# JGCRI/xanthos

Measured on AMD Instinct MI355X. Metric: cell-months/sec (pm_abcd_mrtm, 67,420 cells), higher is better.
Workload: dtype f64

## Files before the change

xanthos_amd/csrc/xh_mrtm_rsum.hip:

```cpp
#include <algorithm>
#include "xh_mrtm_wave_unit.h"

namespace {

__global__ void __launch_bounds__(LANES) __attribute__((amdgpu_waves_per_eu(2, 2))) k_mrtm_rsum(const WaveArgs *ap_) {
    WaveArgsK *ap = (WaveArgsK *)ap_;
    __shared__ __attribute__((aligned(16))) v2d lds[RING * NSLOT];
    __shared__ uint2 xtab[LANES];
    __shared__ unsigned qstage_sh[4 * LANES];
    __shared__ double fend_sh[2 * LANES];
    __shared__ int unit_sh, prio_sh;
    const int unit = wave_claim(ap, &unit_sh, &prio_sh);
    const int prio = prio_sh;
    if (unit < 0) return;
    if (A(months_ready)) {
        if (prio == 3) __builtin_amdgcn_s_setprio(3);
        else if (prio == 1) __builtin_amdgcn_s_setprio(1);
        else __builtin_amdgcn_s_setprio(2);
    } else if (prio == 3) {
        __builtin_amdgcn_s_setprio(3);
    }
    const int p = A(unit_p)[unit];
    const bool has_ghost = A(ghost_edge)[(int64_t)unit * LANES + threadIdx.x] >= 0;
    const bool g = __any(has_ghost), g2 = __any(has_ghost && threadIdx.x >= 8);
    const int nxo = __popcll(__ballot(A(export_edge)[(int64_t)unit * LANES + threadIdx.x] >= 0));
    const bool x = nxo > 0;
    char *l = reinterpret_cast<char *>(lds);
    __attribute__((address_space(3))) unsigned *qst = (__attribute__((address_space(3))) unsigned *)qstage_sh;
    __attribute__((address_space(3))) double *fnd = (__attribute__((address_space(3))) double *)fend_sh;
    fend_sh[threadIdx.x] = 0.0;
    fend_sh[LANES + threadIdx.x] = 0.0;
    if ((p & ~31) != 0x400) {
        if (threadIdx.x == 0) __hip_atomic_store(A(fault), FAULT_PLACE_WAIT, __ATOMIC_RELAXED, __HIP_MEMORY_SCOPE_AGENT);
        return;
    }
    bool bad = false;
#define XH_BY_OUTLETS(...)                                                                 \
    do {                                                                                   \
        if (nxo > 8) wave_unit<__VA_ARGS__, -1>(ap, l, xtab, qst, fnd, unit);              \
        else if (x) wave_unit<__VA_ARGS__, 1>(ap, l, xtab, qst, fnd, unit);                \
        else wave_unit<__VA_ARGS__, 0>(ap, l, xtab, qst, fnd, unit);                       \
    } while (0)
    if (p & 16) {
        if (!(p & 8) || (p & 4)) bad = true;
        else if (g2) XH_BY_OUTLETS(1, 0, 2, true, true, false, 2);
        else if (g) XH_BY_OUTLETS(1, 0, 1, true, true, false, 2);
        else XH_BY_OUTLETS(1, 0, 0, true, true, false, 2);
#undef XH_BY_OUTLETS
    } else if (p & 8) {
        if (p & 4) {
            if (g || !A(fold_cell)) bad = true;
            else wave_unit<1, 0, 0, true, true, true, 1>(ap, l, xtab, qst, fnd, unit);
        } else if (g2) wave_unit<1, 0, 2, true, true, false, 1>(ap, l, xtab, qst, fnd, unit);
        else if (g) wave_unit<1, 0, 1, true, true, false, 1>(ap, l, xtab, qst, fnd, unit);
        else if ((p & 2) || x) wave_unit<1, 0, 0, true, true, false, 1>(ap, l, xtab, qst, fnd, unit);
        else if (p & 1) wave_unit<1, 0, 0, false, true, false, 1>(ap, l, xtab, qst, fnd, unit);
        else wave_unit<0, 0, 0, false, true, false, 1>(ap, l, xtab, qst, fnd, unit);
    } else if (p & 4) {
        if (g || !A(fold_cell)) bad = true;
        else wave_unit<1, 0, 0, true, true, true>(ap, l, xtab, qst, fnd, unit);
    } else if (g2) wave_unit<1, 0, 2, true, true>(ap, l, xtab, qst, fnd, unit);
    else if (g) wave_unit<1, 0, 1, true, true>(ap, l, xtab, qst, fnd, unit);
    else if ((p & 2) || x) wave_unit<1, 0, 0, true, true>(ap, l, xtab, qst, fnd, unit);
    else if (p & 1) wave_unit<1, 0, 0, false, true>(ap, l, xtab, qst, fnd, unit);
    else wave_unit<0, 0, 0, false, true>(ap, l, xtab, qst, fnd, unit);
    if (bad && threadIdx.x == 0)
        __hip_atomic_store(A(fault), FAULT_PLACE_WAIT, __ATOMIC_RELAXED, __HIP_MEMORY_SCOPE_AGENT);
}
#undef A

}

const void *wave_rsum_kernel() { return reinterpret_cast<const void *>(&k_mrtm_rsum); }
```

xanthos_amd/csrc/xh_mrtm_wave.hip:

```cpp
#include <algorithm>
#include "xh_mrtm_wave_unit.h"

namespace {

__global__ void __launch_bounds__(LANES) __attribute__((amdgpu_waves_per_eu(2, 2))) k_mrtm_wave(const WaveArgs *ap_) {
    WaveArgsK *ap = (WaveArgsK *)ap_;
    __shared__ __attribute__((aligned(16))) v2d lds[RING * NSLOT];
    __shared__ uint2 xtab[LANES];
    __shared__ unsigned qstage_sh[2 * LANES];
    __shared__ double fend_sh[LANES];
    __shared__ int unit_sh, prio_sh;
    const int unit = wave_claim(ap, &unit_sh, &prio_sh);
    const int prio = prio_sh;
    if (unit < 0) return;
    if (A(months_ready)) {
        if (prio == 3) __builtin_amdgcn_s_setprio(3);
        else if (prio == 1) __builtin_amdgcn_s_setprio(1);
        else __builtin_amdgcn_s_setprio(2);
    } else if (prio == 3) {
        __builtin_amdgcn_s_setprio(3);
    }
    const int p = A(unit_p)[unit];
    const bool has_ghost = A(ghost_edge)[(int64_t)unit * LANES + threadIdx.x] >= 0;
    const bool g = __any(has_ghost), g2 = __any(has_ghost && threadIdx.x >= 8);
    char *l = reinterpret_cast<char *>(lds);
    __attribute__((address_space(3))) unsigned *qst = (__attribute__((address_space(3))) unsigned *)qstage_sh;
    __attribute__((address_space(3))) double *fnd = (__attribute__((address_space(3))) double *)fend_sh;
    fend_sh[threadIdx.x] = 0.0;
#define WAVE_FORM(PRE, POST, CHAINED, NG1)                                                        \
    case (PRE) | ((POST) << 4) | ((CHAINED) ? 0x100 : 0):                                         \
        if (g2 || (g && !(NG1))) wave_unit<PRE, POST, 2, CHAINED>(ap, l, xtab, qst, fnd, unit);        \
        else if (g) wave_unit<PRE, POST, (NG1) ? 1 : 2, CHAINED>(ap, l, xtab, qst, fnd, unit);         \
        else wave_unit<PRE, POST, 0, CHAINED>(ap, l, xtab, qst, fnd, unit);                            \
        break;
#define WAVE_PAIR(PRE, POST, CHAINED) WAVE_FORM(PRE, POST, CHAINED, false)
#define WAVE_PAIR1(PRE, POST, CHAINED) WAVE_FORM(PRE, POST, CHAINED, true)
    switch (p) {
        WAVE_PAIR1(1, 1, false) WAVE_PAIR1(1, 2, false) WAVE_PAIR1(1, 3, false) WAVE_PAIR1(1, 4, false)
        WAVE_PAIR(2, 1, false) WAVE_PAIR1(2, 2, false) WAVE_PAIR1(2, 3, false) WAVE_PAIR1(2, 4, false)
        WAVE_PAIR(3, 1, false) WAVE_PAIR1(3, 2, false) WAVE_PAIR(3, 3, false) WAVE_PAIR(3, 4, false)
        WAVE_PAIR(4, 1, false) WAVE_PAIR(4, 2, false) WAVE_PAIR(4, 3, false) WAVE_PAIR(4, 4, false)
        WAVE_PAIR(1, 1, true) WAVE_PAIR1(1, 2, true) WAVE_PAIR1(1, 3, true) WAVE_PAIR(1, 4, true)
        WAVE_PAIR(2, 1, true) WAVE_PAIR1(2, 2, true) WAVE_PAIR1(2, 3, true) WAVE_PAIR(2, 4, true)
        default:
            if (threadIdx.x == 0) __hip_atomic_store(A(fault), FAULT_PLACE_WAIT, __ATOMIC_RELAXED, __HIP_MEMORY_SCOPE_AGENT);
    }
#undef WAVE_PAIR1
#undef WAVE_PAIR
#undef WAVE_FORM
}
#undef A

}

const void *wave_exact_kernel() { return reinterpret_cast<const void *>(&k_mrtm_wave); }
```

xanthos_amd/csrc/xh_mrtm_wave_launch.hip:

```cpp
#include <algorithm>
#include "xh_mrtm_wave_unit.h"
#undef A

namespace {

__global__ void k_mrtm_wave_args(WaveArgs a, WaveArgs *dst, uint4 *cnt, unsigned cnt_vec) {
    if (threadIdx.x == 0) *dst = a;
    if (threadIdx.x == 0 && a.months_ready)
        __hip_atomic_store(const_cast<unsigned *>(a.months_ready), a.ready_at_launch, __ATOMIC_RELAXED, __HIP_MEMORY_SCOPE_AGENT);
    for (unsigned i = threadIdx.x; i < cnt_vec; i += blockDim.x) cnt[i] = make_uint4(0u, 0u, 0u, 0u);
}

}

int wave_launch(xh_ctx *ctx, FlowPlan *fp, const FlowSched &s, const FlowIO &io, hipStream_t st, unsigned **place) {
    if (!fp || fp->n_units == 0) return XH_OK;
    if (!fp->skew_ok || fp->max_imports > 8 * SK_R || fp->max_exports > 8 * SK_R || s.ntmin < fp->skew_lmax + 2 * GROUP) {
        if (xh_flow_debug())
            fprintf(stderr, "time-skewed kernel not used: skew_ok %d, imports %d, outlets %d, shortest month %d sub-steps, largest lag %d\n",
                    (int)fp->skew_ok, fp->max_imports, fp->max_exports, s.ntmin, fp->skew_lmax);
        return XH_ERR_LIMIT;
    }
    {
        uint64_t limit = (uint64_t)1 << 32;
// ... 2 lines not shown
        if ((uint64_t)(fp->max_cell + 1) * stride > limit || (io.feed && (int64_t)fp->max_cell >= io.feed->ncell)) {
            if (xh_flow_debug())
                fprintf(stderr, "round-3 time-skewed kernel not used: %d rows x %d months x 8 B exceed its 32-bit row offsets\n",
                        fp->max_cell + 1, s.nmonths);
            return XH_ERR_LIMIT;
        }
    }
    int rs = 2048;
    while (rs < 8 * CH + 4 * fp->skew_lmax || rs < 1024 + (2 * CH + 256) * fp->skew_span) rs *= 2;
    if (const char *env = getenv("XH_FLOW_RS")) {
        const int v = atoi(env);
        if (v >= 2048 && (v & (v - 1)) == 0) rs = v;
    }
    const size_t x_streams = (size_t)std::max(fp->n_edges, 1) * (size_t)rs * sizeof(v2d);
    if (x_streams + (size_t)rs * 16 > ((size_t)1 << 32)) return XH_ERR_LIMIT;
    const size_t x_cnt = ((size_t)(fp->n_edges + fp->n_units + PLACE_WORDS) * sizeof(unsigned) + 255) & ~size_t(255);
    const size_t x_rec0 = ((size_t)(s.nit + 3) * sizeof(MonthRec) + 255) & ~size_t(255);
    const size_t x_rec = x_rec0 + (((size_t)(s.nit + 2) * sizeof(FinRec) + 255) & ~size_t(255));
    if (x_streams + x_cnt + x_rec > fp->x_bytes) {
        if (fp->d_x) {
            XH_HIP(ctx, hipStreamSynchronize(st));
            XH_HIP(ctx, hipFree(fp->d_x));
            fp->d_x = nullptr;
        }
        XH_HIP(ctx, hipMalloc(&fp->d_x, x_streams + x_cnt + x_rec));
        fp->x_bytes = x_streams + x_cnt + x_rec;
        fp->rec_key = 0;
    }
    unsigned *cnt = reinterpret_cast<unsigned *>(static_cast<char *>(fp->d_x) + x_streams);
    MonthRec *d_rec = reinterpret_cast<MonthRec *>(static_cast<char *>(fp->d_x) + x_streams + x_cnt);
    FinRec *d_fin = reinterpret_cast<FinRec *>(static_cast<char *>(fp->d_x) + x_streams + x_cnt + x_rec0);
    const FlowFeed *feed = io.feed;
    auto q_off = [&](int m) -> long long {
        if (!feed) return (long long)m * 8;
        return (long long)(m >> 4) * feed->ncell * 128 + (long long)(m & 15) * 8;
    };
    uint64_t rec_key = XH_FNV_BASIS;
    {
        const long long lay[4] = {s.nit, s.total, feed ? (long long)feed->ncell : -1ll, (long long)(size_t)fp->d_x};
        rec_key = xh_fnv1a(rec_key, lay, sizeof(lay));
        rec_key = xh_fnv1a(rec_key, s.h_m, sizeof(int) * (size_t)s.nit);
        rec_key = xh_fnv1a(rec_key, s.h_nt, sizeof(int) * (size_t)s.nit);
        rec_key = xh_fnv1a(rec_key, s.h_g, sizeof(int) * (size_t)(s.nit + 1));
        rec_key = xh_fnv1a(rec_key, s.h_wr, (size_t)s.nit);
        rec_key = xh_fnv1a(rec_key, s.h_secs, sizeof(double) * (size_t)s.nit);
        if (rec_key == 0) rec_key = 1;
    }
    if (rec_key != fp->rec_key) {
        fp->rec_key = 0;
        fp->h_rec.assign((size_t)(s.nit + 3) * sizeof(MonthRec), 0);
        MonthRec *h = reinterpret_cast<MonthRec *>(fp->h_rec.data());
        for (int it = 0; it < s.nit; ++it) {
            h[it].m = s.h_m[it];
            h[it].nt = s.h_nt[it];
            h[it].g = s.h_g[it];
            h[it].write = s.h_wr[it];
            h[it].secs = s.h_secs[it];
            h[it].q_off = q_off(s.h_m[it]);
        }
        h[s.nit].g = s.total;
        fp->h_fin.assign((size_t)(s.nit + 2) * sizeof(FinRec), 0);
        FinRec *hf = reinterpret_cast<FinRec *>(fp->h_fin.data());
        for (int it = 0; it <= s.nit; ++it) {
            if (it >= 1) {
                hf[it].m_prev_w = h[it - 1].m | (h[it - 1].write ? FIN_WRITE : 0);
                hf[it].nt_prev = h[it - 1].nt;
            }
            hf[it].nt_prev = std::max(hf[it].nt_prev, 1);
            hf[it].secs_next1 = it + 1 < s.nit ? h[it + 1].secs : 1.0;
            hf[it].m_next2 = it + 2 < s.nit ? h[it + 2].m : 0;
            hf[it].q_off_next2 = q_off(hf[it].m_next2);
            hf[it].g_next1 = it + 1 <= s.nit ? h[it + 1].g : s.total;
        }
        hf[s.nit + 1].nt_prev = 1;
        hf[s.nit + 1].secs_next1 = 1.0;
        XH_HIP(ctx, hipMemcpyAsync(d_rec, h, fp->h_rec.size(), hipMemcpyHostToDevice, st));
        XH_HIP(ctx, hipMemcpyAsync(d_fin, hf, fp->h_fin.size(), hipMemcpyHostToDevice, st));
        fp->rec_key = rec_key;
    }

    const int cus = ctx->prop.multiProcessorCount > 0 ? ctx->prop.multiProcessorCount : 256;
    const void *kernel = fp->rsum ? wave_rsum_kernel() : wave_exact_kernel();
    const size_t lds_static = (size_t)RING * NSLOT * sizeof(v2d) + LANES * sizeof(uint2) + 2 * LANES * sizeof(unsigned) +
                              LANES * sizeof(double) + 64 +
                              (fp->rsum ? 2 * LANES * sizeof(unsigned) + LANES * sizeof(double) : 0);
    int n_excl = 0;
    if (fp->rsum && fp->n_special >= 0 && fp->n_pair_units > 0 && xh_env_on("XH_RSUM_EXCL", true))
        n_excl = std::min(fp->n_pair_units, 0xffff);
    int n_wg = 0, resident = 0;
    size_t lds = 0;
    {
        n_wg = fp->n_units + cus;
        if (n_wg > 8 * cus) n_wg = std::max(fp->n_units, 8 * cus);
        {
            const char *env = getenv("XH_FLOW_SPARE");
            if (env) n_wg = fp->n_units + std::max(atoi(env), 0);
        }
        const int per_cu = (n_wg + cus - 1) / cus + 3;
        const size_t share = ((size_t)(160 * 1024) / (size_t)per_cu) & ~size_t(1023);
        lds = share > lds_static + 1024 ? share - lds_static : 0;
        XH_HIP(ctx, hipFuncSetAttribute(kernel, hipFuncAttributeMaxDynamicSharedMemorySize, (int)lds));
        XH_HIP(ctx, hipOccupancyMaxActiveBlocksPerMultiprocessor(&resident, kernel, LANES, lds));
        if ((int64_t)(resident - 1) * cus < n_wg || n_wg > 8 * cus) return XH_ERR_LIMIT;
    }

    WaveArgs a;
    a.cell_of_slot = static_cast<const int *>(fp->d_cell_of_slot.p);
    a.lag = static_cast<const int *>(fp->d_lag.p);
    a.ghost_lag = static_cast<const int *>(fp->d_ghost_lag.p);
    a.export_edge = static_cast<const int *>(fp->d_export_edge.p);
    a.ghost_edge = static_cast<const int *>(fp->d_ghost_edge.p);
    a.edge_cons_unit = static_cast<const int *>(fp->d_edge_cons_unit.p);
    a.ent2 = static_cast<const unsigned *>(fp->d_ent2.p);
    a.eprev = static_cast<const unsigned *>(fp->d_eprev.p);
    a.unit_p = static_cast<const int *>(fp->d_unit_p.p);
    a.unit_order = static_cast<const int *>(fp->d_unit_order.p);
    a.n_units = fp->n_units;
    a.unit_lmax = static_cast<const int *>(fp->d_unit_lmax.p);
    a.unit_glmax = static_cast<const int *>(fp->d_unit_glmax.p);
    a.total_slots = (int64_t)fp->n_units * LANES;
    a.nmonths = s.nmonths;
    a.nit = s.nit;
    a.total = s.total;
    a.odd_ok = s.nt_even ? 0 : 1;
    a.rec = d_rec;
    a.fin = d_fin;
    a.lane_flags = static_cast<const unsigned char *>(fp->d_lane_flags.p);
    a.dt = s.dt;
    a.dtinv = 1.0 / s.dt;
    a.flow_dist = io.flow_dist;
    a.velocity = io.velocity;
    a.area = io.area;
    a.runoff = feed ? feed->q_staged : io.runoff;
    a.q_row_stride = feed ? 128u : (unsigned)s.nmonths * 8u;
    a.ready_at_launch = feed ? feed->ready_at_launch : UINT_MAX;
    a.months_ready = feed ? feed->months_ready : nullptr;
    a.place_epoch = feed ? feed->place_epoch : nullptr;
    a.epoch = feed ? feed->epoch : 0u;
    a.n_excl = n_excl;
    a.fenced = xh_env_on("XH_ROUTE_FENCED", false) ? 1 : 0;
    a.S0 = io.S0;
    a.chs = io.chs;
    a.avg = io.avg;
    a.S_end = io.S_end;
    a.F_end = io.F_end;
    a.xbuf = static_cast<char *>(fp->d_x);
    a.xbytes = (unsigned)x_streams;
    a.ring_mask_b = (unsigned)rs * 16u - 1u;
    a.rs = rs;
    a.ready = cnt;
    a.done = cnt + fp->n_edges;
    a.place = cnt + fp->n_edges + fp->n_units;
    *place = a.place;
    unsigned *fault = nullptr;
    int rc = xh_fault_word(ctx, &fault);
    if (rc) return rc;
    a.fault = fault;
    if (s.test_fault) XH_HIP(ctx, hipMemsetD32Async(reinterpret_cast<hipDeviceptr_t>(fault), (int)FAULT_TEST, 1, st));
    a.stats = nullptr;
    {
        const char *env = getenv("XH_FLOW_STATS");
        if (env && env[0] == '1') {
            if (!fp->d_stats) XH_HIP(ctx, hipMalloc(reinterpret_cast<void **>(&fp->d_stats), (size_t)fp->n_units * 48));
            a.stats = fp->d_stats;
        }
    }
    a.fold_cell = static_cast<const int *>(fp->d_fold_cell.p);
// ... 12 lines not shown
```

xanthos_amd/csrc/xh_mrtm_wave_unit.h:

```cpp
#pragma once
#include <algorithm>
#include <climits>
#include <cstdlib>
#include <type_traits>

#include "xh_mrtm_flow.h"

namespace {


constexpr int LANES = 64;
constexpr int SK_P = 4;
#ifndef XH_WAVE_MIDZONE
#define XH_WAVE_MIDZONE 1
#endif
#ifndef XH_WAVE_BMOV
#define XH_WAVE_BMOV 1
#endif
constexpr int NSLOT = 2 * LANES + 1;
constexpr int RING = 8;
constexpr int GROUP = 16;
constexpr int SK_R = 2;
#ifndef XH_WAVE_CH
#define XH_WAVE_CH 256
// ... 36 lines not shown
    int odd_ok;
    const MonthRec *rec;
    const FinRec *fin;
    double dt, dtinv;
    const double *flow_dist, *velocity, *area, *runoff, *S0;
    double *chs, *avg, *S_end, *F_end;
    unsigned q_row_stride;
    unsigned ready_at_launch;
    const unsigned *months_ready;
    unsigned *place_epoch;
    unsigned epoch;
    int n_excl;
    int fenced;
    char *xbuf;
    unsigned xbytes;
    unsigned ring_mask_b;
    int rs;
    unsigned *ready;
    unsigned *done;
    unsigned *fault;
    unsigned long long *stats;
    const int *fold_cell;
};

__device__ __forceinline__ unsigned ld_relaxed(const unsigned *p) {
    return __hip_atomic_load(p, __ATOMIC_RELAXED, __HIP_MEMORY_SCOPE_AGENT);
}

constexpr unsigned long long SPIN_LIMIT_TICKS = 500000000ull;

__device__ __forceinline__ bool wave_wait_ge(bool need, const unsigned *p, unsigned target, unsigned &seen,
                                             unsigned *fault, unsigned code) {
    bool ok = !need || seen >= target;
    if (__all(ok)) return true;
    const unsigned long long t0 = __builtin_amdgcn_s_memrealtime();
    for (;;) {
        if (!ok) {
            seen = ld_relaxed(p);
            ok = seen >= target;
        }
        if (__all(ok)) return true;
        if (ld_relaxed(fault) != 0) return false;
        if (__builtin_amdgcn_s_memrealtime() - t0 > SPIN_LIMIT_TICKS) {
            __hip_atomic_store(fault, code, __ATOMIC_RELAXED, __HIP_MEMORY_SCOPE_AGENT);
            return false;
        }
        __builtin_amdgcn_s_sleep(4);
    }
}

typedef double v2d __attribute__((ext_vector_type(2)));
typedef unsigned v4u __attribute__((ext_vector_type(4)));
constexpr int AUX_SC1 = 16;
typedef __attribute__((address_space(3))) const char lds_cchar;
typedef __attribute__((address_space(3))) char lds_char;

typedef __attribute__((address_space(4))) const WaveArgs WaveArgsK;
template <class T>
__device__ __forceinline__ T xh_ldarg(__attribute__((address_space(4))) const T *p) {
    asm volatile("" : "+s"(p));
    return *p;
}
#define A(f) xh_ldarg(&ap->f)

template <bool ONE> struct Val;
template <> struct Val<false> {
    typedef v2d T;
    typedef __attribute__((address_space(3))) const v2d lds_c;
    typedef __attribute__((address_space(3))) v2d lds_m;
    static constexpr unsigned B = 16;
    static __device__ __forceinline__ T zero() { return v2d{0.0, 0.0}; }
};
template <> struct Val<true> {
    typedef double T;
    typedef __attribute__((address_space(3))) const double lds_c;
    typedef __attribute__((address_space(3))) double lds_m;
    static constexpr unsigned B = 8;
    static __device__ __forceinline__ T zero() { return 0.0; }
};

template <int PRE, int POST, int NG, bool CHAIN, bool RSUM = false, bool FOLD = false, int SGL = 0, int NXR = -1>
__device__ __forceinline__ void wave_unit(WaveArgsK *ap, char *lds_generic, uint2 *xtab,
                                          __attribute__((address_space(3))) unsigned *qstage,
                                          __attribute__((address_space(3))) double *fend, const int unit) {
    constexpr bool HAS_G = NG > 0;
    constexpr bool V8 = SGL == 1;
    typedef Val<V8> V;
    typedef typename V::T val_t;
    typedef typename V::lds_c lds_cv;
    typedef typename V::lds_m lds_mv;
    constexpr unsigned VB = V::B;
    constexpr unsigned SLOTB = NSLOT * VB;
    lds_char *lds0 = (lds_char *)lds_generic;
    const int lane = threadIdx.x;
    const int64_t slot = (int64_t)unit * LANES + lane;

    const int gc = A(cell_of_slot)[slot];
    const bool valid = gc >= 0;
    const int gc_safe = valid ? gc : 0;
    const unsigned row_off = (unsigned)gc_safe * A(q_row_stride);
    const double tauinv = valid ? A(velocity)[gc] / A(flow_dist)[gc] : 0.0;
    const double acoef = 1.0 - tauinv * A(dt);
    const double area = valid ? A(area)[gc] : 0.0;
    const double S0v = (valid && A(S0)) ? A(S0)[gc] : 0.0;
    auto ent_off = [](unsigned o) { return V8 ? o >> 1 : o; };
    static_assert(!RSUM || (PRE <= 1 && POST == 0), "reassociated form: one inflow entry");
    static_assert(!FOLD || (RSUM && NG == 0), "folded leaves: reassociated form, units without imports");
    static_assert(SGL == 0 || RSUM, "single-sum plans: reassociated form");
    const int gcL = FOLD ? A(fold_cell)[slot] : -1;
    const bool validL = FOLD && valid && gcL >= 0;
    const unsigned row_offL = (unsigned)(validL ? gcL : 0) * A(q_row_stride);
    const double tauL = validL ? A(velocity)[gcL] / A(flow_dist)[gcL] : 0.0;
    const double acoefL = 1.0 - tauL * A(dt);
    const double areaL = validL ? A(area)[gcL] : 0.0;
    const double S0L = (validL && A(S0)) ? A(S0)[gcL] : 0.0;
    double SL = 0.0, favgL = 0.0, erlL = 0.0, erlL_n = 0.0, snapSL = 0.0, snapAL = 0.0, FL = 0.0;
    constexpr double FOLD_EPS = 1e-6;
    unsigned gfold = (validL && !(tauL * A(dt) <= 1.0 - 1.0 / 1048576.0 && tauL >= 0.0 && S0L >= 0.0)) ? 1u : 0u;
    constexpr double SGL_EPS = 1e-6;
    constexpr double SGL_XEPS = 1e-10;
    unsigned gsgl = 0;
    bool xlane = false;
    double fmin_seen = 0.0;
    if (SGL != 0) {
        const unsigned lf = A(lane_flags)[slot];
        xlane = valid && (lf & 2u) != 0;
        gsgl = (valid && (!(tauinv >= 0.0) || (!(tauinv * A(dt) <= 1.0 - 1.0 / 1048576.0) && !(lf & 1u)) || S0v < 0.0)) ? 1u : 0u;
    }
    constexpr int PRE_N = PRE > 0 ? PRE : 1, POST_N = POST > 0 ? POST : 1;
    lds_cchar *epre[PRE_N], *epost[POST_N];
#pragma unroll
    for (int w = 0; w < PRE; ++w) epre[w] = lds0 + ent_off(A(ent2)[(int64_t)w * A(total_slots) + slot]);
#pragma unroll
    for (int w = 0; w < POST; ++w) epost[w] = lds0 + ent_off(A(ent2)[(int64_t)(SK_P + w) * A(total_slots) + slot]);
    lds_cchar *eprv = lds0 + (CHAIN ? ent_off(A(eprev)[slot]) : 0u);
    lds_mv *own = (lds_mv *)lds0 + lane;
    const int xedge = A(export_edge)[slot];
    const int gedge = A(ghost_edge)[slot];
    const bool has_x = xedge >= 0, has_g = gedge >= 0;
    const unsigned long long xmask = __ballot(has_x), gmask = __ballot(has_g);
    const int nx_out = __popcll(xmask), ng = __popcll(gmask);
    static_assert(NXR >= -1 && NXR <= 1, "outlet rounds known at compile time: none or one");
    const bool any_x = NXR < 0 ? xmask != 0 : NXR > 0, any_g = HAS_G;
    const int lmax = A(unit_lmax)[unit], glmax = A(unit_glmax)[unit];
    const int lag_g = has_g ? A(ghost_lag)[slot] : 0;
    const unsigned *ready_p = A(ready) + (has_g ? gedge : 0);
    const unsigned *done_p = A(done) + (has_x ? A(edge_cons_unit)[xedge] : 0);
    const unsigned maskb = A(ring_mask_b);
    const unsigned oob = ~maskb;
    const __amdgpu_buffer_rsrc_t xr = __builtin_amdgcn_make_buffer_rsrc(A(xbuf), 0, (int)A(xbytes), 0x00020000);
    const int total = A(total), nit = A(nit);
    const bool odd_ok = A(odd_ok) != 0;

    if (has_x) xtab[__popcll(xmask & ((1ull << lane) - 1ull))] = make_uint2((unsigned)lane, (unsigned)xedge);
    const int sub = lane & 7, grp = lane >> 3;
    const bool x2 = NXR < 0 && nx_out > 8;
    unsigned gfull[SK_R], xbyte[SK_R];
    lds_mv *gdst[SK_R];
    lds_cv *xsrc[SK_R];
#pragma unroll
    for (int r = 0; r < SK_R; ++r) {
        const int k = r * 8 + grp;
        const bool gon = k < ng, xon = k < nx_out;
        const int ge = gon ? A(ghost_edge)[(int64_t)unit * LANES + k] : 0;
        const int gl = gon ? A(ghost_lag)[(int64_t)unit * LANES + k] : 0;
        gfull[r] = gon ? ((unsigned)ge * (maskb + 1u)) | (((unsigned)(sub - gl) * 16u) & maskb) : oob;
// ... 34 lines not shown
        MonthRec r;
        r.m = p_rec[i].m;
        r.nt = p_rec[i].nt;
        r.g = p_rec[i].g;
        r.write = p_rec[i].write;
        r.secs = p_rec[i].secs;
        r.q_off = p_rec[i].q_off;
        return r;
    };
    const int nmo = A(nmonths);
    const unsigned q_lds = (unsigned)(size_t)qstage;
    auto runoff_fetch = [&](long long q_off) {
        const char *src = reinterpret_cast<const char *>(p_runoff) + q_off + (size_t)row_off;
        unsigned keep;
        asm volatile("s_mov_b32 %0, m0\n\ts_mov_b32 m0, %2\n\tglobal_load_lds_dword %1, off\n\ts_add_u32 m0, m0, 252\n\t"
                     "global_load_lds_dword %1, off offset:4\n\ts_mov_b32 m0, %0"
                     : "=&s"(keep)
                     : "v"(src), "s"(q_lds)
                     : "memory");
        if (FOLD) {
            const char *srcL = reinterpret_cast<const char *>(p_runoff) + q_off + (size_t)row_offL;
            asm volatile("s_mov_b32 %0, m0\n\ts_mov_b32 m0, %2\n\tglobal_load_lds_dword %1, off\n\ts_add_u32 m0, m0, 252\n\t"
                         "global_load_lds_dword %1, off offset:4\n\ts_mov_b32 m0, %0"
                         : "=&s"(keep)
                         : "v"(srcL), "s"(q_lds + 2u * LANES * 4u)
                         : "memory");
        }
    };
    auto runoff_take = [&]() {
        if (any_x || any_g) asm volatile("s_waitcnt vmcnt(4)" ::: "memory");
        else asm volatile("s_waitcnt vmcnt(0)" ::: "memory");
        const unsigned lo = qstage[lane], hi = qstage[LANES + lane];
        return __hiloint2double((int)hi, (int)lo);
    };
    double erl_n = 0.0;
    {
        const MonthRec r0 = ld_rec(0), r1 = ld_rec(1);
        auto ld_q = [&](long long q_off) {
            return *reinterpret_cast<const double *>(reinterpret_cast<const char *>(p_runoff) + q_off + (size_t)row_off);
        };
        const double q0 = ld_q(r0.q_off);
        erl_n = ((valid ? q0 : 0.0) * area) * 1000.0 / r0.secs;
        if (RSUM) erl_n *= A(dt);
        if (SGL != 0) gsgl |= (erl_n < -SGL_EPS) ? 2u : 0u;
        if (FOLD) {
            const double q0L = *reinterpret_cast<const double *>(reinterpret_cast<const char *>(p_runoff) + r0.q_off + (size_t)row_offL);
            erlL_n = (((validL ? q0L : 0.0) * areaL) * 1000.0 / r0.secs) * A(dt);
        }
        if (nit > 1) runoff_fetch(r1.q_off);
    }
    constexpr int OB = 4;
    double ob_s[OB], ob_a[OB];
    double ob_sL[FOLD ? OB : 1], ob_aL[FOLD ? OB : 1];
#pragma unroll
    for (int j = 0; j < OB; ++j) ob_s[j] = ob_a[j] = 0.0;
#pragma unroll
    for (int j = 0; j < (FOLD ? OB : 1); ++j) ob_sL[j] = ob_aL[j] = 0.0;
    bool alive = true;
    unsigned mready = A(ready_at_launch);
    auto wait_months = [&](unsigned need) {
        const unsigned *p = A(months_ready);
        if (!p) return true;
        const unsigned long long t0 = __builtin_amdgcn_s_memrealtime();
        for (;;) {
            unsigned v = 0;
            if (lane == 0) v = __hip_atomic_fetch_add(const_cast<unsigned *>(p), 0u, __ATOMIC_RELAXED, __HIP_MEMORY_SCOPE_AGENT);
            v = (unsigned)__builtin_amdgcn_readfirstlane((int)v);
            if (v >= need) {
                mready = v;
                return true;
            }
            if (ld_relaxed(A(fault)) != 0) return false;
            if (__builtin_amdgcn_s_memrealtime() - t0 > SPIN_LIMIT_TICKS) {
                __hip_atomic_store(A(fault), FAULT_DATA_WAIT, __ATOMIC_RELAXED, __HIP_MEMORY_SCOPE_AGENT);
                return false;
            }
            __builtin_amdgcn_s_sleep(16);
        }
    };
    unsigned long long cyc_wait_data = 0, cyc_wait_ring = 0, zone_groups = 0;
    const unsigned long long cyc_begin = __builtin_amdgcn_s_memtime();
    const unsigned long long rt_begin = __builtin_amdgcn_s_memrealtime();

    unsigned seen_ready = 0, seen_done = 0, pend_ready = 0, pend_done = 0;
    auto load_async = [&](const unsigned *q) {
        unsigned v;
        asm volatile("global_load_dword %0, %1, off sc1" : "=v"(v) : "v"(q) : "memory");
        return v;
    };
    auto check = [&](int n) {
        const unsigned long long w0 = __builtin_amdgcn_s_memtime();
        asm volatile("s_waitcnt vmcnt(8)" : "+v"(pend_ready), "+v"(pend_done) : : "memory");
        asm volatile("s_waitcnt vmcnt(0)" ::: "memory");
        if (SGL == 2) gsgl |= (xlane && fmin_seen < -SGL_XEPS) ? 4u : 0u;
        if ((FOLD && __any(gfold != 0)) || (SGL != 0 && __any(gsgl != 0))) {
            __hip_atomic_store(A(fault), FAULT_GUARD, __ATOMIC_RELAXED, __HIP_MEMORY_SCOPE_AGENT);
            alive = false;
        }
        const bool fenced = A(fenced) == 1;
        if (any_x) {
            const int pub = min(max(n - RING - lmax, 0), total);
            if (fenced) __builtin_amdgcn_fence(__ATOMIC_RELEASE, "agent");
            if (has_x) __hip_atomic_store(A(ready) + xedge, (unsigned)pub, __ATOMIC_RELAXED, __HIP_MEMORY_SCOPE_AGENT);
            const int need = n + CH - lmax - A(rs);
            seen_done = max(seen_done, pend_done);
            if (need > 0 && alive)
                alive = wave_wait_ge(has_x, done_p, (unsigned)min(need, total), seen_done, A(fault), FAULT_RING_WAIT);
        }
        const unsigned long long w1 = __builtin_amdgcn_s_memtime();
        if (any_g && alive) {
            if (lane == 0)
                __hip_atomic_store(A(done) + unit, (unsigned)min(max(n - glmax, 0), total), __ATOMIC_RELAXED,
                                   __HIP_MEMORY_SCOPE_AGENT);
            const int need = min(total, n + CH + GROUP - lag_g);
            seen_ready = max(seen_ready, pend_ready);
            alive = wave_wait_ge(has_g && need > 0, ready_p, (unsigned)max(need, 0), seen_ready, A(fault), FAULT_DATA_WAIT);
            if (fenced) __builtin_amdgcn_fence(__ATOMIC_ACQUIRE, "agent");
            asm volatile("" ::: "memory");
        }
        if (any_x) pend_done = load_async(done_p);
        if (any_g) pend_ready = load_async(ready_p);
        cyc_wait_ring += w1 - w0;
        cyc_wait_data += __builtin_amdgcn_s_memtime() - w1;
    };

    auto finalize = [&](int it) {
        const FinRec f = fc;
        fc = ld_fin(it + 1 <= nit ? it + 1 : nit + 1);
        if (it + 1 < nit) {
            const double qn = runoff_take();
            erl_n = ((valid ? qn : 0.0) * area) * 1000.0 / f.secs_next1;
            if (RSUM) erl_n *= dt;
            if (SGL != 0) gsgl |= (erl_n < -SGL_EPS) ? 2u : 0u;
            if (FOLD) {
                const unsigned lo = qstage[2 * LANES + lane], hi = qstage[3 * LANES + lane];
                const double qnL = __hiloint2double((int)hi, (int)lo);
                erlL_n = (((validL ? qnL : 0.0) * areaL) * 1000.0 / f.secs_next1) * dt;
            }
        }
        if (it >= 1) {
            const int m = f.m_prev_w & (FIN_WRITE - 1);
            const bool write_prev = (f.m_prev_w & FIN_WRITE) != 0;
#pragma unroll
            for (int j = 0; j < OB - 1; ++j) {
                ob_s[j] = ob_s[j + 1];
                ob_a[j] = ob_a[j + 1];
            }
            ob_s[OB - 1] = snapS;
            ob_a[OB - 1] = snapA / (double)f.nt_prev;
            if (FOLD) {
#pragma unroll
                for (int j = 0; j < OB - 1; ++j) {
                    ob_sL[j] = ob_sL[j + 1];
                    ob_aL[j] = ob_aL[j + 1];
                }
                ob_sL[OB - 1] = snapSL;
                ob_aL[OB - 1] = snapAL / (double)f.nt_prev;
                gfold |= (snapSL < -FOLD_EPS) ? 2u : 0u;
                if (write_prev && validL) {
                    if ((m & (OB - 1)) == OB - 1) {
                        const int64_t o = (int64_t)gcL * nmo + (m - (OB - 1));
#pragma unroll
                        for (int j = 0; j < OB; j += 2) {
                            if (p_chs) *reinterpret_cast<v2d *>(p_chs + o + j) = v2d{ob_sL[j], ob_sL[j + 1]};
                            if (p_avg) *reinterpret_cast<v2d *>(p_avg + o + j) = v2d{ob_aL[j], ob_aL[j + 1]};
                        }
                    } else if (m == nmo - 1) {
                        const int r = (m & (OB - 1)) + 1;
                        const int64_t o = (int64_t)gcL * nmo + (m + 1 - r);
#pragma unroll
                        for (int j = 0; j < OB; ++j)
                            if (j >= OB - r) {
                                if (p_chs) p_chs[o + j - (OB - r)] = ob_sL[j];
                                if (p_avg) p_avg[o + j - (OB - r)] = ob_aL[j];
                            }
                    }
                }
            }
            if (write_prev && valid) {
                if ((m & (OB - 1)) == OB - 1) {
                    const int64_t o = (int64_t)gc * nmo + (m - (OB - 1));
#pragma unroll
                    for (int j = 0; j < OB; j += 2) {
                        if (p_chs) *reinterpret_cast<v2d *>(p_chs + o + j) = v2d{ob_s[j], ob_s[j + 1]};
                        if (p_avg) *reinterpret_cast<v2d *>(p_avg + o + j) = v2d{ob_a[j], ob_a[j + 1]};
                    }
                } else if (m == nmo - 1) {
                    const int r = (m & (OB - 1)) + 1;
                    const int64_t o = (int64_t)gc * nmo + (m + 1 - r);
#pragma unroll
                    for (int j = 0; j < OB; ++j)
                        if (j >= OB - r) {
                            if (p_chs) p_chs[o + j - (OB - r)] = ob_s[j];
                            if (p_avg) p_avg[o + j - (OB - r)] = ob_a[j];
                        }
                }
            }
        }
        if (it + 2 < nit) {
            if ((unsigned)f.m_next2 >= mready) alive = wait_months((unsigned)f.m_next2 + 1u);
            if (alive) runoff_fetch(f.q_off_next2);
        }
        return f.g_next1;
    };
// ... 180 lines not shown
    }
    unsigned long long prof_plain = 0;
#else
#define PROF_MARK(acc)
#endif
    auto housekeeping = [&](int n) {
        if (n > 0 && (n & (CH - 1)) == 0) check(n);
        if (alive && n == nf) {
            const int g_next = finalize(itf);
            ++itf;
            nf = itf <= nit ? ((g_next + lmax + 1 + GROUP - 1) & ~(GROUP - 1)) : INT_MAX;
        }
        PROF_MARK(prof_fin)
    };
    int n = 0;
    while (n < N && alive) {
        if (itz <= nit && n + GROUP > gz && n <= gz + lmax) {
            const int edge = itz == 0 ? 1 : (itz == nit ? 2 : 0);
            auto zone_run = [&](auto mid_c) {
                do {
                    housekeeping(n);
                    if (!alive) break;
                    ++zone_groups;
                    const int rel = nx - n;
#pragma unroll
                    for (int j = 0; j < GROUP; ++j) substep(std::true_type(), mid_c, n, j, edge, rel);
                    n += GROUP;
                    PROF_MARK(prof_zone)
                } while (n <= gz + lmax && n < N);
            };
#if XH_WAVE_MIDZONE
            if (edge == 0 && !odd_ok) zone_run(std::true_type());
            else zone_run(std::false_type());
#else
            zone_run(std::false_type());
#endif
            if (alive) {
                nx = itz < nit ? nx + ntz : INT_MAX;
                ++itz;
                gz = p_rec[itz <= nit ? itz : nit].g;
                if (itz > nit) gz = INT_MAX;
                ntz = p_rec[itz <= nit ? itz : nit].nt;
            }
        } else {
            const int n_end = itz <= nit ? min(N, gz & ~(GROUP - 1)) : N;
            do {
                housekeeping(n);
                if (!alive) break;
#pragma unroll
                for (int j = 0; j < GROUP; ++j) substep(std::false_type(), std::false_type(), n, j, 0, 0);
                n += GROUP;
                PROF_MARK(prof_plain)
            } while (n < n_end);
        }
    }
    if (alive) {
        while (itf <= nit) finalize(itf++);
        if (SGL == 2) gsgl |= (xlane && fmin_seen < -SGL_XEPS) ? 4u : 0u;
        if ((FOLD && __any(gfold != 0)) || (SGL != 0 && __any(gsgl != 0))) {
            __hip_atomic_store(A(fault), FAULT_GUARD, __ATOMIC_RELAXED, __HIP_MEMORY_SCOPE_AGENT);
            alive = false;
        }
    }
    if (alive) {
        if (any_x) {
            const unsigned xpos = ((unsigned)(N - RING - lmax) * 16u) & maskb;
            store_pair(*xsrc[0], xbyte[0], xpos);
            if (x2) store_pair(*xsrc[1], xbyte[1], xpos);
            asm volatile("s_waitcnt vmcnt(0)" ::: "memory");
            if (A(fenced) == 1) __builtin_amdgcn_fence(__ATOMIC_RELEASE, "agent");
            if (has_x) __hip_atomic_store(A(ready) + xedge, (unsigned)total, __ATOMIC_RELAXED, __HIP_MEMORY_SCOPE_AGENT);
        }
        if (any_g && lane == 0)
            __hip_atomic_store(A(done) + unit, (unsigned)total, __ATOMIC_RELAXED, __HIP_MEMORY_SCOPE_AGENT);
        if (valid) {
            if (A(S_end)) A(S_end)[gc] = snapS;
            if (A(F_end)) A(F_end)[gc] = fend[lane];
        }
        if (validL) {
            if (A(S_end)) A(S_end)[gcL] = snapSL;
            if (A(F_end)) A(F_end)[gcL] = fend[LANES + lane];
        }
    }
    const bool guard_set = __any((gfold | gsgl) != 0);
    if (A(stats) && lane == 0) {
        unsigned long long *st = A(stats) + (int64_t)unit * 6;
        const unsigned long long cyc = __builtin_amdgcn_s_memtime() - cyc_begin;
        st[0] = cyc - cyc_wait_data - cyc_wait_ring;
        st[1] = cyc;
        st[2] = __builtin_amdgcn_s_memrealtime() - rt_begin;
        const unsigned hw = __builtin_amdgcn_s_getreg((4) | (0 << 6) | (31 << 11));
        const unsigned xcc = __builtin_amdgcn_s_getreg((20) | (0 << 6) | (3 << 11));
        st[3] = (unsigned long long)((PRE + POST + (CHAIN ? 1 : 0) + 1) & 15) | (any_g ? 16u : 0u) | (any_x ? 32u : 0u) |
                (V8 ? 64u : 0u) | (guard_set ? 128u : 0u) | ((unsigned long long)hw << 8) | ((unsigned long long)(xcc & 15u) << 40) |
                (zone_groups << 44);
        st[4] = cyc_wait_data;
        st[5] = cyc_wait_ring;
#ifdef XH_WAVE_PROFILE
        st[0] = prof_plain;
        st[4] = prof_zone;
        st[5] = prof_fin;
#endif
    }
}


__device__ __forceinline__ int wave_claim(WaveArgsK *ap, int *unit_sh_p, int *prio_sh_p) {
    int &unit_sh = *unit_sh_p, &prio_sh = *prio_sh_p;
    if (threadIdx.x == 0) {
        prio_sh = 0;
        unsigned *pl = A(place);
        const unsigned hw = __builtin_amdgcn_s_getreg((4) | (0 << 6) | (31 << 11));
        const unsigned xcc = __builtin_amdgcn_s_getreg((20) | (0 << 6) | (3 << 11)) & 15u;
        const unsigned key = ((((xcc * 8u + ((hw >> 13) & 7u)) * 2u + ((hw >> 12) & 1u)) * 16u + ((hw >> 8) & 15u)) * 4u) +
                             ((hw >> 4) & 3u);
        unsigned *pl_cu = pl + 16 + PLACE_KEYS + (key >> 2);
        const int n_units = A(n_units);
        const unsigned n_wg = gridDim.x;
        unsigned *fault = A(fault);
        auto wait_for = [&](unsigned *word, unsigned target) {
            const unsigned long long t0 = __builtin_amdgcn_s_memrealtime();
            while (__hip_atomic_load(word, __ATOMIC_ACQUIRE, __HIP_MEMORY_SCOPE_AGENT) < target) {
                if (ld_relaxed(fault) != 0 || __builtin_amdgcn_s_memrealtime() - t0 > SPIN_LIMIT_TICKS) {
                    __hip_atomic_store(fault, FAULT_PLACE_WAIT, __ATOMIC_RELAXED, __HIP_MEMORY_SCOPE_AGENT);
                    return false;
                }
                __builtin_amdgcn_s_sleep(8);
            }
            return true;
        };
        auto add = [&](int word) { return __hip_atomic_fetch_add(pl + word, 1u, __ATOMIC_RELAXED, __HIP_MEMORY_SCOPE_AGENT); };
        const unsigned rank = __hip_atomic_fetch_add(pl + 16 + key, 1u, __ATOMIC_RELAXED, __HIP_MEMORY_SCOPE_AGENT) & 0xffffu;
        bool leader = false;
        unsigned cu_rank = 0;
        if (rank == 0) {
            add(2);
            cu_rank = __hip_atomic_fetch_add(pl_cu, 1u, __ATOMIC_RELAXED, __HIP_MEMORY_SCOPE_AGENT) & 0xffffu;
            leader = cu_rank == 0u;
            if (leader) add(9);
        } else if (rank == 1) {
            add(1);
        }
        const unsigned registered = __hip_atomic_fetch_add(pl + 0, 1u, __ATOMIC_RELEASE, __HIP_MEMORY_SCOPE_AGENT);
        if (registered + 1u == n_wg && A(place_epoch))
            __hip_atomic_store(A(place_epoch), A(epoch), __ATOMIC_RELAXED, __HIP_MEMORY_SCOPE_AGENT);
        int idx = -1;
        if (wait_for(pl + 0, n_wg)) {
            const int firsts = (int)ld_relaxed(pl + 2), seconds = (int)ld_relaxed(pl + 1), leaders = (int)ld_relaxed(pl + 9);
            const int n_excl = A(n_excl);
            int ncu = min(n_excl, leaders);
            ncu = max(min(ncu, (seconds - max(n_units - firsts, 0)) / 7), 0);
            bool excl_cu = false;
            int displaced = 0, claimed = 0;
            bool ok = true;
            if (ncu > 0) {
                if (leader) {
                    if ((int)add(10) < ncu) {
                        const int cnt = (int)(ld_relaxed(pl_cu) & 0xffffu);
                        const int base = (int)add(13);
                        if (base < n_excl) {
                            __hip_atomic_fetch_or(pl_cu, 0x10000u, __ATOMIC_RELAXED, __HIP_MEMORY_SCOPE_AGENT);
                            __hip_atomic_fetch_add(pl + 11, (unsigned)(cnt - 1), __ATOMIC_RELAXED, __HIP_MEMORY_SCOPE_AGENT);
                            idx = n_units - 1 - base;
                        }
                    }
                    __hip_atomic_fetch_add(pl + 12, 1u, __ATOMIC_RELEASE, __HIP_MEMORY_SCOPE_AGENT);
                }
                ok = wait_for(pl + 12, (unsigned)leaders);
                excl_cu = (ld_relaxed(pl_cu) & 0x10000u) != 0;
                displaced = (int)ld_relaxed(pl + 11);
                claimed = min((int)ld_relaxed(pl + 13), n_excl);
            }
            const int nx = claimed;
            const int firsts_eff = firsts - displaced;
            const int need2 = max(n_units - firsts_eff, 0);
            if (idx >= 0 || !ok) {
            } else if (rank >= 2) {
                idx = -2;
// ... 31 lines not shown
```

Baseline: 3.176 billion.

## Stage async progress-counter loads through LDS and specialize single-unit rsum outlets

The asynchronous polls of the neighbour ready/done counters now use global_load_lds_dword into a new LDS staging buffer, not VGPR-returning loads, which frees registers and removes the inline-asm register ties that held them live across the wait. The check step reads the staged values back from LDS, and a final vmcnt(0) drain is added before exit. Separately, the rsum kernel now also dispatches single-group (SGL=1) units through the outlet-count specializations, which adds template instantiations and code size. The LDS staging adds M0 save/restore overhead and a small LDS footprint, and the static-LDS size accounting is updated to match.

```diff
diff --git a/xanthos_amd/csrc/xh_mrtm_rsum.hip b/xanthos_amd/csrc/xh_mrtm_rsum.hip
--- a/xanthos_amd/csrc/xh_mrtm_rsum.hip
+++ b/xanthos_amd/csrc/xh_mrtm_rsum.hip
@@ -1,5 +1,13 @@
 #include <algorithm>
 #include "xh_mrtm_wave_unit.h"
+
+#define XH_SGL_FOLD 1
+#define XH_SGL_NG0 2
+#define XH_SGL_NG1 4
+#define XH_SGL_NG2 8
+#ifndef XH_RSUM_SGL_NXR
+#define XH_RSUM_SGL_NXR (XH_SGL_FOLD | XH_SGL_NG0 | XH_SGL_NG1 | XH_SGL_NG2)
+#endif
 
 namespace {
 
@@ -8,6 +16,7 @@
     __shared__ __attribute__((aligned(16))) v2d lds[RING * NSLOT];
     __shared__ uint2 xtab[LANES];
     __shared__ unsigned qstage_sh[4 * LANES];
+    __shared__ unsigned cstage_sh[2 * LANES];
     __shared__ double fend_sh[2 * LANES];
     __shared__ int unit_sh, prio_sh;
     const int unit = wave_claim(ap, &unit_sh, &prio_sh);
@@ -27,6 +36,7 @@
     const bool x = nxo > 0;
     char *l = reinterpret_cast<char *>(lds);
     __attribute__((address_space(3))) unsigned *qst = (__attribute__((address_space(3))) unsigned *)qstage_sh;
+    __attribute__((address_space(3))) unsigned *cst = (__attribute__((address_space(3))) unsigned *)cstage_sh;
     __attribute__((address_space(3))) double *fnd = (__attribute__((address_space(3))) double *)fend_sh;
     fend_sh[threadIdx.x] = 0.0;
     fend_sh[LANES + threadIdx.x] = 0.0;
@@ -37,33 +47,39 @@
     bool bad = false;
 #define XH_BY_OUTLETS(...)                                                                 \
     do {                                                                                   \
-        if (nxo > 8) wave_unit<__VA_ARGS__, -1>(ap, l, xtab, qst, fnd, unit);              \
-        else if (x) wave_unit<__VA_ARGS__, 1>(ap, l, xtab, qst, fnd, unit);                \
-        else wave_unit<__VA_ARGS__, 0>(ap, l, xtab, qst, fnd, unit);                       \
+        if (nxo > 8) wave_unit<__VA_ARGS__, -1>(ap, l, xtab, qst, cst, fnd, unit);         \
+        else if (x) wave_unit<__VA_ARGS__, 1>(ap, l, xtab, qst, cst, fnd, unit);           \
+        else wave_unit<__VA_ARGS__, 0>(ap, l, xtab, qst, cst, fnd, unit);                  \
     } while (0)
     if (p & 16) {
         if (!(p & 8) || (p & 4)) bad = true;
         else if (g2) XH_BY_OUTLETS(1, 0, 2, true, true, false, 2);
         else if (g) XH_BY_OUTLETS(1, 0, 1, true, true, false, 2);
         else XH_BY_OUTLETS(1, 0, 0, true, true, false, 2);
-#undef XH_BY_OUTLETS
     } else if (p & 8) {
+#define XH_SGL_BY_OUTLETS(BIT, ...)                                                        \
+    do {                                                                                   \
+        if constexpr (((XH_RSUM_SGL_NXR) & (BIT)) != 0) XH_BY_OUTLETS(__VA_ARGS__);        \
+        else wave_unit<__VA_ARGS__>(ap, l, xtab, qst, cst, fnd, unit);                     \
+    } while (0)
         if (p & 4) {
             if (g || !A(fold_cell)) bad = true;
-            else wave_unit<1, 0, 0, true, true, true, 1>(ap, l, xtab, qst, fnd, unit);
-        } else if (g2) wave_unit<1, 0, 2, true, true, false, 1>(ap, l, xtab, qst, fnd, unit);
-        else if (g) wave_unit<1, 0, 1, true, true, false, 1>(ap, l, xtab, qst, fnd, unit);
-        else if ((p & 2) || x) wave_unit<1, 0, 0, true, true, false, 1>(ap, l, xtab, qst, fnd, unit);
-        else if (p & 1) wave_unit<1, 0, 0, false, true, false, 1>(ap, l, xtab, qst, fnd, unit);
-        else wave_unit<0, 0, 0, false, true, false, 1>(ap, l, xtab, qst, fnd, unit);
+            else XH_SGL_BY_OUTLETS(XH_SGL_FOLD, 1, 0, 0, true, true, true, 1);
+        } else if (g2) XH_SGL_BY_OUTLETS(XH_SGL_NG2, 1, 0, 2, true, true, false, 1);
+        else if (g) XH_SGL_BY_OUTLETS(XH_SGL_NG1, 1, 0, 1, true, true, false, 1);
+        else if ((p & 2) || x) XH_SGL_BY_OUTLETS(XH_SGL_NG0, 1, 0, 0, true, true, false, 1);
+#undef XH_SGL_BY_OUTLETS
+#undef XH_BY_OUTLETS
+        else if (p & 1) wave_unit<1, 0, 0, false, true, false, 1>(ap, l, xtab, qst, cst, fnd, unit);
+        else wave_unit<0, 0, 0, false, true, false, 1>(ap, l, xtab, qst, cst, fnd, unit);
     } else if (p & 4) {
         if (g || !A(fold_cell)) bad = true;
-        else wave_unit<1, 0, 0, true, true, true>(ap, l, xtab, qst, fnd, unit);
-    } else if (g2) wave_unit<1, 0, 2, true, true>(ap, l, xtab, qst, fnd, unit);
-    else if (g) wave_unit<1, 0, 1, true, true>(ap, l, xtab, qst, fnd, unit);
-    else if ((p & 2) || x) wave_unit<1, 0, 0, true, true>(ap, l, xtab, qst, fnd, unit);
-    else if (p & 1) wave_unit<1, 0, 0, false, true>(ap, l, xtab, qst, fnd, unit);
-    else wave_unit<0, 0, 0, false, true>(ap, l, xtab, qst, fnd, unit);
+        else wave_unit<1, 0, 0, true, true, true>(ap, l, xtab, qst, cst, fnd, unit);
+    } else if (g2) wave_unit<1, 0, 2, true, true>(ap, l, xtab, qst, cst, fnd, unit);
+    else if (g) wave_unit<1, 0, 1, true, true>(ap, l, xtab, qst, cst, fnd, unit);
+    else if ((p & 2) || x) wave_unit<1, 0, 0, true, true>(ap, l, xtab, qst, cst, fnd, unit);
+    else if (p & 1) wave_unit<1, 0, 0, false, true>(ap, l, xtab, qst, cst, fnd, unit);
+    else wave_unit<0, 0, 0, false, true>(ap, l, xtab, qst, cst, fnd, unit);
     if (bad && threadIdx.x == 0)
         __hip_atomic_store(A(fault), FAULT_PLACE_WAIT, __ATOMIC_RELAXED, __HIP_MEMORY_SCOPE_AGENT);
 }
diff --git a/xanthos_amd/csrc/xh_mrtm_wave.hip b/xanthos_amd/csrc/xh_mrtm_wave.hip
--- a/xanthos_amd/csrc/xh_mrtm_wave.hip
+++ b/xanthos_amd/csrc/xh_mrtm_wave.hip
@@ -9,6 +9,7 @@
     __shared__ uint2 xtab[LANES];
     __shared__ unsigned qstage_sh[2 * LANES];
     __shared__ double fend_sh[LANES];
+    __shared__ unsigned cstage_sh[2 * LANES];
     __shared__ int unit_sh, prio_sh;
     const int unit = wave_claim(ap, &unit_sh, &prio_sh);
     const int prio = prio_sh;
@@ -26,12 +27,13 @@
     char *l = reinterpret_cast<char *>(lds);
     __attribute__((address_space(3))) unsigned *qst = (__attribute__((address_space(3))) unsigned *)qstage_sh;
     __attribute__((address_space(3))) double *fnd = (__attribute__((address_space(3))) double *)fend_sh;
+    __attribute__((address_space(3))) unsigned *cst = (__attribute__((address_space(3))) unsigned *)cstage_sh;
     fend_sh[threadIdx.x] = 0.0;
 #define WAVE_FORM(PRE, POST, CHAINED, NG1)                                                        \
     case (PRE) | ((POST) << 4) | ((CHAINED) ? 0x100 : 0):                                         \
-        if (g2 || (g && !(NG1))) wave_unit<PRE, POST, 2, CHAINED>(ap, l, xtab, qst, fnd, unit);        \
-        else if (g) wave_unit<PRE, POST, (NG1) ? 1 : 2, CHAINED>(ap, l, xtab, qst, fnd, unit);         \
-        else wave_unit<PRE, POST, 0, CHAINED>(ap, l, xtab, qst, fnd, unit);                            \
+        if (g2 || (g && !(NG1))) wave_unit<PRE, POST, 2, CHAINED>(ap, l, xtab, qst, cst, fnd, unit);        \
+        else if (g) wave_unit<PRE, POST, (NG1) ? 1 : 2, CHAINED>(ap, l, xtab, qst, cst, fnd, unit);         \
+        else wave_unit<PRE, POST, 0, CHAINED>(ap, l, xtab, qst, cst, fnd, unit);                            \
         break;
 #define WAVE_PAIR(PRE, POST, CHAINED) WAVE_FORM(PRE, POST, CHAINED, false)
 #define WAVE_PAIR1(PRE, POST, CHAINED) WAVE_FORM(PRE, POST, CHAINED, true)
diff --git a/xanthos_amd/csrc/xh_mrtm_wave_launch.hip b/xanthos_amd/csrc/xh_mrtm_wave_launch.hip
--- a/xanthos_amd/csrc/xh_mrtm_wave_launch.hip
+++ b/xanthos_amd/csrc/xh_mrtm_wave_launch.hip
@@ -108,7 +108,7 @@
     const int cus = ctx->prop.multiProcessorCount > 0 ? ctx->prop.multiProcessorCount : 256;
     const void *kernel = fp->rsum ? wave_rsum_kernel() : wave_exact_kernel();
     const size_t lds_static = (size_t)RING * NSLOT * sizeof(v2d) + LANES * sizeof(uint2) + 2 * LANES * sizeof(unsigned) +
-                              LANES * sizeof(double) + 64 +
+                              2 * LANES * sizeof(unsigned) + LANES * sizeof(double) + 64 +
                               (fp->rsum ? 2 * LANES * sizeof(unsigned) + LANES * sizeof(double) : 0);
     int n_excl = 0;
     if (fp->rsum && fp->n_special >= 0 && fp->n_pair_units > 0 && xh_env_on("XH_RSUM_EXCL", true))
diff --git a/xanthos_amd/csrc/xh_mrtm_wave_unit.h b/xanthos_amd/csrc/xh_mrtm_wave_unit.h
--- a/xanthos_amd/csrc/xh_mrtm_wave_unit.h
+++ b/xanthos_amd/csrc/xh_mrtm_wave_unit.h
@@ -142,6 +142,7 @@
 template <int PRE, int POST, int NG, bool CHAIN, bool RSUM = false, bool FOLD = false, int SGL = 0, int NXR = -1>
 __device__ __forceinline__ void wave_unit(WaveArgsK *ap, char *lds_generic, uint2 *xtab,
                                           __attribute__((address_space(3))) unsigned *qstage,
+                                          __attribute__((address_space(3))) unsigned *cstage,
                                           __attribute__((address_space(3))) double *fend, const int unit) {
     constexpr bool HAS_G = NG > 0;
     constexpr bool V8 = SGL == 1;
@@ -342,15 +343,20 @@
     const unsigned long long cyc_begin = __builtin_amdgcn_s_memtime();
     const unsigned long long rt_begin = __builtin_amdgcn_s_memrealtime();
 
-    unsigned seen_ready = 0, seen_done = 0, pend_ready = 0, pend_done = 0;
-    auto load_async = [&](const unsigned *q) {
-        unsigned v;
-        asm volatile("global_load_dword %0, %1, off sc1" : "=v"(v) : "v"(q) : "memory");
-        return v;
+    unsigned seen_ready = 0, seen_done = 0;
+    cstage[lane] = 0u;
+    cstage[LANES + lane] = 0u;
+    const unsigned c_lds = (unsigned)(size_t)cstage;
+    auto load_async = [&](const unsigned *q, unsigned half) {
+        unsigned keep;
+        asm volatile("s_mov_b32 %0, m0\n\ts_mov_b32 m0, %2\n\ts_nop 0\n\tglobal_load_lds_dword %1, off sc1\n\ts_mov_b32 m0, %0"
+                     : "=&s"(keep)
+                     : "v"(q), "s"(c_lds + half * (unsigned)(LANES * 4))
+                     : "memory");
     };
     auto check = [&](int n) {
         const unsigned long long w0 = __builtin_amdgcn_s_memtime();
-        asm volatile("s_waitcnt vmcnt(8)" : "+v"(pend_ready), "+v"(pend_done) : : "memory");
+        asm volatile("s_waitcnt vmcnt(8)" ::: "memory");
         asm volatile("s_waitcnt vmcnt(0)" ::: "memory");
         if (SGL == 2) gsgl |= (xlane && fmin_seen < -SGL_XEPS) ? 4u : 0u;
         if ((FOLD && __any(gfold != 0)) || (SGL != 0 && __any(gsgl != 0))) {
@@ -363,7 +369,7 @@
             if (fenced) __builtin_amdgcn_fence(__ATOMIC_RELEASE, "agent");
             if (has_x) __hip_atomic_store(A(ready) + xedge, (unsigned)pub, __ATOMIC_RELAXED, __HIP_MEMORY_SCOPE_AGENT);
             const int need = n + CH - lmax - A(rs);
-            seen_done = max(seen_done, pend_done);
+            seen_done = max(seen_done, cstage[lane]);
             if (need > 0 && alive)
                 alive = wave_wait_ge(has_x, done_p, (unsigned)min(need, total), seen_done, A(fault), FAULT_RING_WAIT);
         }
@@ -373,13 +379,13 @@
                 __hip_atomic_store(A(done) + unit, (unsigned)min(max(n - glmax, 0), total), __ATOMIC_RELAXED,
                                    __HIP_MEMORY_SCOPE_AGENT);
             const int need = min(total, n + CH + GROUP - lag_g);
-            seen_ready = max(seen_ready, pend_ready);
+            seen_ready = max(seen_ready, cstage[LANES + lane]);
             alive = wave_wait_ge(has_g && need > 0, ready_p, (unsigned)max(need, 0), seen_ready, A(fault), FAULT_DATA_WAIT);
             if (fenced) __builtin_amdgcn_fence(__ATOMIC_ACQUIRE, "agent");
             asm volatile("" ::: "memory");
         }
-        if (any_x) pend_done = load_async(done_p);
-        if (any_g) pend_ready = load_async(ready_p);
+        if (any_x) load_async(done_p, 0u);
+        if (any_g) load_async(ready_p, 1u);
         cyc_wait_ring += w1 - w0;
         cyc_wait_data += __builtin_amdgcn_s_memtime() - w1;
     };
@@ -726,6 +732,7 @@
             if (A(F_end)) A(F_end)[gcL] = fend[LANES + lane];
         }
     }
+    asm volatile("s_waitcnt vmcnt(0)" ::: "memory");
     const bool guard_set = __any((gfold | gsgl) != 0);
     if (A(stats) && lane == 0) {
         unsigned long long *st = A(stats) + (int64_t)unit * 6;
@@ -736,8 +743,9 @@
         const unsigned hw = __builtin_amdgcn_s_getreg((4) | (0 << 6) | (31 << 11));
         const unsigned xcc = __builtin_amdgcn_s_getreg((20) | (0 << 6) | (3 << 11));
         st[3] = (unsigned long long)((PRE + POST + (CHAIN ? 1 : 0) + 1) & 15) | (any_g ? 16u : 0u) | (any_x ? 32u : 0u) |
-                (V8 ? 64u : 0u) | (guard_set ? 128u : 0u) | ((unsigned long long)hw << 8) | ((unsigned long long)(xcc & 15u) << 40) |
-                (zone_groups << 44);
+                (V8 ? 64u : 0u) | (guard_set ? 128u : 0u) | ((unsigned long long)(hw & 0xffffu) << 8) |
+                ((unsigned long long)ng << 24) | ((unsigned long long)nx_out << 31) | (FOLD ? 1ull << 38 : 0ull) |
+                (NXR >= 0 ? 1ull << 39 : 0ull) | ((unsigned long long)(xcc & 15u) << 40) | (zone_groups << 44);
         st[4] = cyc_wait_data;
         st[5] = cyc_wait_ring;
 #ifdef XH_WAVE_PROFILE
```

New measurement: 3.186 billion, median of 4. About the same (+0.3%).
